# LeiXu84/fireFoam-dev

Hardware: AMD Instinct MI355X
Metric: PIMPLE outer-iterations/sec on 64M-cell hex mesh; pEqn SpMV GB/s vs HBM peak (higher is better)
Workload: dtype f64; 1 GPU; synthetic 400^3 hex box (64000000 cells), buoyant plume + 5-species EDC-shaped source, PIMPLE 1/2/0: rhoEqn + UEqn + YEEqn(4 Yi + h) + 2 pEqn per step; cells=64000000, faces=191520000, parallelism=1 GPU, transport_solvers=PBiCGStab+DILU

## Files before the change

firefoam-dev_amd/binding.py:

```python
import ctypes as C
import os
import re
import subprocess

import numpy as np

_HERE = os.path.dirname(os.path.abspath(__file__))
_ROOT = os.path.dirname(_HERE)
_SO = os.path.join(_HERE, "lib", "libffm.so")
_HDR = os.path.join(_ROOT, "include", "ffm.h")

SOLVERS = {"PCG": 0, "PBiCGStab": 1, "PBiCG": 2, "diagonal": 3, "smoothSolver": 4}
PRECONDS = {"none": 0, "DIC": 1, "DILU": 2, "GaussSeidel": 3, "symGaussSeidel": 4, "diagonal": 5}


class FfmError(RuntimeError):
    pass


class Perf(C.Structure):
    _fields_ = [("initialResidual", C.c_double), ("finalResidual", C.c_double),
                ("nIterations", C.c_int), ("converged", C.c_int), ("singular", C.c_int)]

    def as_dict(self):
# ... 69 lines not shown
        "ffm_ldu_bind_coeffs_native_d": ([vp, dp, dp, dp, C.c_int], C.c_int),
        "ffm_ldu_set_interfaces": ([vp, C.c_int, ip, C.POINTER(ip), C.POINTER(hp), C.POINTER(hp), ip], C.c_int),
        "ffm_ldu_set_global_cells": ([vp, C.c_long], C.c_int),
        "ffm_ldu_global_cells": ([vp], C.c_long),
        "ffm_spmv": ([vp, dp, dp], C.c_int),
        "ffm_tmul": ([vp, dp, dp], C.c_int),
        "ffm_sumA": ([vp, dp], C.c_int),
        "ffm_residual": ([vp, dp, dp, dp], C.c_int),
        "ffm_precond_setup": ([vp, C.c_int, dp], C.c_int),
        "ffm_precond_apply": ([vp, C.c_int, C.c_int, dp, dp], C.c_int),
        "ffm_precond_setup_multi": ([vp, C.c_int, C.c_int, C.POINTER(C.c_void_p), C.POINTER(C.c_void_p)], C.c_int),
        "ffm_ldu_tile_reach": ([vp, C.POINTER(C.c_int), C.POINTER(C.c_int), C.POINTER(C.c_int)], C.c_int),
        "ffm_gs_smooth": ([vp, C.c_int, C.c_int, dp, dp], C.c_int),
        "ffm_solve_d": ([vp, C.c_int, C.c_int, C.c_double, C.c_double, C.c_int, C.c_int, C.c_int, dp, dp,
                         C.POINTER(Perf)], C.c_int),
        "ffm_solve": ([vp, C.c_int, C.c_int, C.c_double, C.c_double, C.c_int, C.c_int, C.c_int, hp, hp,
                       C.POINTER(Perf)], C.c_int),
        "ffm_solve_multi_d": ([vp, C.c_int, C.c_int, C.c_int, C.c_double, C.c_double, C.c_int, C.c_int, C.POINTER(C.c_void_p), dp, dp,
                               C.POINTER(C.c_void_p), C.POINTER(C.c_void_p), C.POINTER(Perf)], C.c_int),
        "ffm_ldu_unbind_coeffs": ([vp], C.c_int),
        "ffm_ldu_offdiag_epoch": ([vp], C.c_ulong),
        "ffm_ldu_tile_coef_read": ([vp, C.c_int, hp], C.c_int),
        "ffm_ldu_tile_gathers": ([vp], C.c_long),
        "ffm_ldu_tile_code_bytes": ([vp, C.c_int, C.POINTER(C.c_long), C.POINTER(C.c_long)], C.c_int),
        "ffm_tile_share_codes": ([C.c_int, C.POINTER(C.c_long), ip, C.POINTER(C.c_ushort), C.c_long, C.c_int, C.c_long, C.POINTER(C.c_uint),
                                  C.POINTER(C.c_ushort), C.c_long, C.POINTER(C.c_long), C.POINTER(C.c_long)], C.c_int),
        "ffm_debug_pool_poison": ([vp, C.c_int], C.c_int),
        "ffm_bench_spmv": ([vp, dp, dp, C.c_int, hp], C.c_int),
        "ffm_bench_precond": ([vp, C.c_int, dp, dp, C.c_int, hp], C.c_int),
        "ffm_debug_set_sweep_ticket": ([vp, C.c_uint], C.c_int),
        "ffm_ldu_set_exchange_tags": ([vp, C.c_int, C.c_int, ip], C.c_int),
        "ffm_field_binary": ([vp, C.c_int, C.c_long, dp, dp, dp], C.c_int),
        "ffm_field_scalar": ([vp, C.c_int, C.c_long, dp, C.c_double, C.c_int, dp], C.c_int),
        "ffm_field_unary": ([vp, C.c_int, C.c_long, dp, dp], C.c_int),
        "ffm_field_eval": ([vp, C.c_long, C.c_int, C.POINTER(C.c_void_p), C.c_int, hp, C.c_int, C.POINTER(C.c_ushort), dp], C.c_int),
        "ffm_reduce_sum": ([vp, dp, C.c_long, hp], C.c_int),
        "ffm_reduce_min": ([vp, dp, C.c_long, hp], C.c_int),
        "ffm_reduce_max": ([vp, dp, C.c_long, hp], C.c_int),
        "ffm_reduce_dot": ([vp, dp, dp, C.c_long, hp], C.c_int),
        "ffm_reduce_summag": ([vp, dp, C.c_long, hp], C.c_int),
        "ffm_mesh_create": ([vp, hp, hp, hp, hp, hp, hp, C.c_int, ip, C.POINTER(ip), C.POINTER(hp), C.POINTER(hp), C.POINTER(vp)], C.c_int),
        "ffm_mesh_destroy": ([vp], C.c_int),
        "ffm_mesh_set_face_centres": ([vp, hp], C.c_int),
        "ffm_mesh_set_nonorth_correction": ([vp, hp], C.c_int),
        "ffm_pyro_create": ([vp, C.c_int, C.c_int, C.c_double, C.c_double, C.c_double, C.c_double, C.POINTER(vp)], C.c_int),
        "ffm_pyro_set_solids": ([vp, hp, hp], C.c_int),
# ... 484 lines not shown
    def face_map(self):
        m = np.empty(self.nFaces, np.int32)
        _check(lib().ffm_ldu_get_face_map(self.h, _ip(m)), "ffm_ldu_get_face_map")
        return m

    def bind_coeffs_native(self, diag, upper, lower=None, offDiagUnchanged=False):
        self._bound = (diag, upper, lower)
        _check(lib().ffm_ldu_bind_coeffs_native_d(self.h, C.c_void_p(diag.data_ptr()), C.c_void_p(upper.data_ptr()),
                                                  None if lower is None else C.c_void_p(lower.data_ptr()), 1 if offDiagUnchanged else 0),
               "ffm_ldu_bind_coeffs_native_d")
        return self

    def unbind_coeffs(self):
        _check(lib().ffm_ldu_unbind_coeffs(self.h), "ffm_ldu_unbind_coeffs")
        self._bound = None
        return self

    def tile_coef(self, which):
        self.ctx._ready()
        out = np.empty(3 * self.nOwned, np.float64)
        _check(lib().ffm_ldu_tile_coef_read(self.h, which, _hp(out)), "ffm_ldu_tile_coef_read")
        return out

    def tile_gathers(self):
        return int(lib().ffm_ldu_tile_gathers(self.h))

    def tile_code_bytes(self, which):
        u, t = C.c_long(), C.c_long()
        _check(lib().ffm_ldu_tile_code_bytes(self.h, which, C.byref(u), C.byref(t)), "ffm_ldu_tile_code_bytes")
        return u.value, t.value

    @property
    def offdiag_epoch(self):
        return int(lib().ffm_ldu_offdiag_epoch(self.h))

    def debug_set_sweep_ticket(self, value):
        _check(lib().ffm_debug_set_sweep_ticket(self.h, int(value) & 0xFFFFFFFF), "ffm_debug_set_sweep_ticket")

    @property
    def native_order(self):
        return bool(lib().ffm_ldu_is_native_order(self.h))

    def cell_order(self):
        o = np.empty(self.nCells, np.int32)
        _check(lib().ffm_ldu_get_cell_order(self.h, _ip(o)), "ffm_ldu_get_cell_order")
        return o
# ... 582 lines not shown
```

firefoam-dev_amd/csrc/ffm_internal.hpp:

```cpp
#pragma once
#include <hip/hip_runtime.h>
#include <string>
#include <tuple>
#include <unordered_map>

#include "ffm_host.hpp"

struct ncclComm;
struct ffm_tile_plan;

#define FFM_HIP(call)                                                            \
    do {                                                                         \
        hipError_t e_ = (call);                                                  \
        if (e_ != hipSuccess) {                                                  \
            ffm_set_error("%s:%d %s -> %s", __FILE__, __LINE__, #call,           \
                          hipGetErrorString(e_));                                \
            return FFM_ERR_HIP;                                                  \
        }                                                                        \
    } while (0)

constexpr int RED_THREADS = 256;
constexpr int RED_BLOCKS = 2048;
constexpr int NSCAL = 64;

// ... 96 lines not shown
    int upWidthUniform = -1;
    int loWidthUniform = -1;
    int maxW = 0;
    int loShift = 4;
    int *upOff = nullptr, *loOff = nullptr;
    int *upNbr = nullptr;
    int *loEnt = nullptr;
    int *flowOrder = nullptr;
    int *cellPerm = nullptr;
    int *faceSrc = nullptr;
    std::vector<int> h_callerToNative;
    std::vector<int> h_upOff, h_loOff, h_loEnt, h_upNbr;
    int *callerToNative = nullptr;

    double *diag = nullptr, *upper = nullptr, *lower = nullptr;
    double *lowerBuf = nullptr;

    int *rowSched = nullptr; int nSched = 0;

    double *rD = nullptr;
    int rDKind = -1;
    unsigned long coeffEpoch = 0, rDEpoch = ~0ul;
    unsigned long offDiagEpoch = 0;
    bool directPending = false;
    const double *directUpper = nullptr, *directLower = nullptr;
    unsigned long tileGathers = 0;
    double *diagBuf = nullptr, *upperBuf = nullptr;

    std::vector<double *> work;
    double *gsProd = nullptr;
    double *permIn[3] = {nullptr, nullptr, nullptr};

    std::vector<ffm_iface> ifaces;
    std::vector<int> ifaceTags, ghTags;
    int haloTotal = 0;
    int *ifFaceCells = nullptr;
    double *ifBou = nullptr, *ifInt = nullptr;
    double *haloSend = nullptr, *haloRecv = nullptr;
    double *haloSend_h = nullptr, *haloRecv_h = nullptr;
    int nIfCells = 0;
    int *ifCell = nullptr, *ifCellStart = nullptr, *ifItem = nullptr;

    std::vector<int> ghNbrRank, ghSendOff, ghRecvOff;
    int *ghSendCells = nullptr;
    bool ghPending = false;
    double *ghSendBuf = nullptr, *ghSendBuf_h = nullptr, *ghRecvBuf_h = nullptr;
// ... 32 lines not shown
int ffm_tile_gs_ghost_terms(ffm_ldu *A, const double *psi, double *bP);
int ffm_ghost_exchange(ffm_ldu *A, double *x);
int ffm_ghost_exchange_begin(ffm_ldu *A, double *x);
int ffm_ghost_exchange_split(ffm_ldu *A, const double *sendFrom, double *ghostInto);
int ffm_ghost_exchange_end(ffm_ldu *A);
int ffm_tile_gs(ffm_ldu *A, bool sym, double *psi, const double *bP, double *bSave, double *prod3);
bool ffm_tile_amul_usable(const ffm_ldu *A);
int ffm_tile_amul(ffm_ldu *A, const double *x, double *y, int dotSlot, const ffm_scal_op &t = ffm_scal_op());
void ffm_tile_free(ffm_ldu *A);
bool ffm_tile_usable(const ffm_ldu *A);
struct FfmFvSegs { int nSeg; const int4 *seg; const int4 *rec; };
bool ffm_tile_fv_segments(ffm_ldu *A, int runLength, FfmFvSegs *out);
bool ffm_tile_coef_direct_ok(const ffm_ldu *A);
int ffm_tile_coef_direct(ffm_ldu *A, bool lower, double **fU, double **fL, double **bU);
void ffm_tile_coef_written(ffm_ldu *A, const double *upper_d, const double *lower_d);
void ffm_tile_coef_adopt(ffm_ldu *A);
bool ffm_tile_pcg_fusable(const ffm_ldu *A);
int ffm_tile_pcg_fwd(ffm_ldu *A, double *rA, double *wA, int slot, const double *qA = nullptr, const ffm_scal_op &t = ffm_scal_op());
bool ffm_tile_amul_pcg_usable(const ffm_ldu *A);
bool ffm_tile_amul_asym_usable(const ffm_ldu *A);
int ffm_tile_amul_asym(ffm_ldu *A, const double *x, double *y);
int ffm_tile_amul_pcg(ffm_ldu *A, const double *w, const double *pin, double *pout, double *psi, double *y, int dotSlot, const ffm_scal_op &t = ffm_scal_op());
int ffm_tile_pcg_bwd(ffm_ldu *A, const double *rA, double *wA, int slot, const ffm_scal_op &t = ffm_scal_op());
#define FFM_TILE_MAXSYS 5
bool ffm_tile_multi_fits(const ffm_ldu *A, int n);
int ffm_tile_precond(ffm_ldu *A, int precond, bool transpose, int n, const double *const *rD, const double *const *r, double *const *w);
int ffm_tile_calc_rD(ffm_ldu *A, int n, const double *const *diag, double *const *D);
int ffm_k_spmv_multi(ffm_ldu *A, int n, const double *const *diag, const double *const *x, double *const *y, double *const *sumA);
extern "C" int ffm_solve_internal_i(ffm_ldu *A, int solver, int precond, double tol, double relTol, int minIter, int maxIter, int nSweeps,
                                    double *psi, const double *source, ffm_perf *perf);
int ffm_gs_smooth_i(ffm_ldu *A, bool sym, int nSweeps, double *psi, const double *b);
int ffm_halo_exchange(ffm_ldu *A, const double *x);
int ffm_ghost_exchange(ffm_ldu *A, double *x);
int ffm_read_scalars(ffm_ctx *ctx);

int ffm_k_dot(ffm_ctx *ctx, const double *x, const double *y, long n, int slot, const ffm_scal_op &t = ffm_scal_op());
int ffm_k_summag(ffm_ctx *ctx, const double *x, long n, int slot, const ffm_scal_op &t = ffm_scal_op());
int ffm_k_sum(ffm_ctx *ctx, const double *x, long n, int slot, const ffm_scal_op &t = ffm_scal_op());
int ffm_k_sumsqr(ffm_ctx *ctx, const double *x, long n, int slot, const ffm_scal_op &t = ffm_scal_op());

static inline int ffm_grid(long n, int threads) { return (int)((n + threads - 1) / threads); }
```

firefoam-dev_amd/csrc/ffm_ldu.hip:

```cpp
#include "ffm_internal.hpp"
#include "ffm_device.hpp"
#include <algorithm>

template <class T>
static int upload(ffm_ctx *c, T **dst, const std::vector<T> &v, size_t minCount = 1)
{
    size_t n = std::max(v.size(), minCount);
    FFM_HIP(hipMalloc((void **)dst, n * sizeof(T)));
    if (!v.empty()) FFM_HIP(hipMemcpyAsync(*dst, v.data(), v.size() * sizeof(T), hipMemcpyHostToDevice, c->stream));
    return FFM_OK;
}

extern "C" int ffm_ldu_create(ffm_ctx *ctx, int N, int F, const int *l, const int *u, ffm_ldu **out)
{ return ffm_ldu_create_ext(ctx, N, 0, F, l, u, out); }

extern "C" int ffm_ldu_create_ext(ffm_ctx *ctx, int nOwn, int nGhost, int F, const int *l, const int *u, ffm_ldu **out)
{ return ffm_ldu_create_hint(ctx, nOwn, nGhost, F, l, u, nullptr, out); }

static int ldu_create_impl(ffm_ctx *ctx, int nOwn, int nGhost, int F, const int *l, const int *u, const int *groupHint, int forceMode,
                           ffm_ldu **out);

extern "C" int ffm_ldu_create_hint(ffm_ctx *ctx, int nOwn, int nGhost, int F, const int *l, const int *u, const int *groupHint,
                                   ffm_ldu **out)
{
// ... 65 lines not shown
    A->nSlices = L.nSlices; A->upTotal = L.upTotal; A->loTotal = L.loTotal;
    A->upWidthUniform = L.upWidthUniform; A->loWidthUniform = L.loWidthUniform; A->maxW = L.maxW; A->loShift = L.loShift;
    A->h_upOff = L.upOff; A->h_loOff = L.loOff;
    A->h_callerToNative = std::move(L.callerToNative);
    const int rc = ldu_upload(A, a, L);
    if (rc) { ffm_ldu_destroy(A); return rc; }
    *out = A;
    return FFM_OK;
}

extern "C" int ffm_ldu_destroy(ffm_ldu *A)
{
    if (!A) return FFM_OK;
    hipSetDevice(A->ctx->device);
    hipStreamSynchronize(A->ctx->stream);
    for (double *w : A->work) hipFree(w);
    hipFree(A->gsProd);
    for (int i = 0; i < 3; i++) hipFree(A->permIn[i]);
    hipFree(A->upOff); hipFree(A->loOff); hipFree(A->upNbr); hipFree(A->loEnt); hipFree(A->faceSrc);
    hipFree(A->cellPerm); hipFree(A->callerToNative); hipFree(A->flowOrder);
    hipFree(A->grpCell); hipFree(A->sweepTicket); hipFree(A->rowSched);
    ffm_tile_free(A);
    hipFree(A->ghSendCells); hipFree(A->ghSendBuf); if (A->ghSendBuf_h) hipHostFree(A->ghSendBuf_h); if (A->ghRecvBuf_h) hipHostFree(A->ghRecvBuf_h);
    hipFree(A->diagBuf); hipFree(A->upperBuf); hipFree(A->lowerBuf); hipFree(A->rD);
    hipFree(A->ifFaceCells); hipFree(A->ifBou); hipFree(A->ifInt); hipFree(A->haloSend); hipFree(A->haloRecv);
    hipFree(A->ifCell); hipFree(A->ifCellStart); hipFree(A->ifItem);
    delete A;
    return FFM_OK;
}

extern "C" int ffm_ldu_ncells(const ffm_ldu *A) { return A ? A->nCells : FFM_ERR_ARG; }
extern "C" int ffm_ldu_sweep_mode(const ffm_ldu *A) { return !A ? FFM_ERR_ARG : A->sweepMode; }
extern "C" int ffm_ldu_nowned(const ffm_ldu *A) { return A ? A->nOwned : FFM_ERR_ARG; }
extern "C" int ffm_ldu_nfaces(const ffm_ldu *A) { return A ? A->nFaces : FFM_ERR_ARG; }
extern "C" int ffm_ldu_nlevels(const ffm_ldu *A) { return A ? A->nLevels : FFM_ERR_ARG; }
extern "C" int ffm_ldu_is_native_order(const ffm_ldu *A) { return A ? (A->identity ? 1 : 0) : FFM_ERR_ARG; }
extern "C" int ffm_ldu_get_cell_order(const ffm_ldu *A, int *newToOld)
{
    if (!A || !newToOld) return FFM_ERR_ARG;
    std::copy(A->h_newToOldCell.begin(), A->h_newToOldCell.end(), newToOld);
    return FFM_OK;
}
extern "C" int ffm_ldu_n_native_faces(const ffm_ldu *A) { return A ? A->upTotal : FFM_ERR_ARG; }
extern "C" int ffm_ldu_get_face_map(const ffm_ldu *A, int *callerToNative)
{
    if (!A || !callerToNative) return FFM_ERR_ARG;
    std::copy(A->h_callerToNative.begin(), A->h_callerToNative.end(), callerToNative);
// ... 419 lines not shown
```

firefoam-dev_amd/csrc/ffm_solve.hip:

```cpp
#include "ffm_internal.hpp"
#include "ffm_device.hpp"
#include <algorithm>
#include <cmath>
#include <cstring>


__global__ void k_scalar_op(double *s, int op, double arg, int iter, int in)
{
    if (threadIdx.x || blockIdx.x) return;
    scalar_op_body(s, op, arg, iter, in);
}

static int scalar_op(ffm_ctx *c, int op, double arg = 0.0, int iter = 0, int in = S_TMP0)
{
    hipLaunchKernelGGL(k_scalar_op, dim3(1), dim3(64), 0, c->stream, c->scal_d, op, arg, iter, in);
    FFM_HIP(hipGetLastError());
    return FFM_OK;
}
static ffm_scal_op tail_op(ffm_ctx *c, int op, double arg = 0.0, int iter = 0)
{
    ffm_scal_op t; t.op = op; t.arg = arg; t.iter = iter; t.fused = c->nRanks == 1 && !c->comm;
    return t;
}
static int finish_dot(ffm_ctx *c, const ffm_scal_op &t, int nSlots = 1)
// ... 346 lines not shown
        unsigned int z = 0;
        ffm_h2d(A->ctx, A->sweepTicket + 1, &z, sizeof(z));
        return FFM_ERR_HIP;
    }
    return FFM_OK;
}

static int calc_rD(ffm_ldu *A)
{
    if (A->sweepMode == 2) {
        const double *dg = A->diag;
        return ffm_tile_calc_rD(A, 1, &dg, &A->rD);
    }
    FlowArgs a; FFM_TRY(flow_args(A, SM_RD, a));
    FLOW_LAUNCH(SM_RD, a);
    FFM_HIP(hipGetLastError());
    return FFM_OK;
}

int ffm_precond_setup_i(ffm_ldu *A, int precond)
{
    if (A->rDKind == precond && A->rDEpoch == A->coeffEpoch) return FFM_OK;
    hipStream_t s = A->ctx->stream;
    switch (precond) {
    case FFM_NONE: break;
    case FFM_DIC:
        if (!A->symmetric) { ffm_set_error("DIC needs a symmetric matrix"); return FFM_ERR_UNSUPPORTED; }
        FFM_TRY(calc_rD(A)); break;
    case FFM_DILU: FFM_TRY(calc_rD(A)); break;
    case FFM_DIAGONALP:
        hipLaunchKernelGGL(k_recip, dim3(sgrid(A->nOwned)), dim3(256), 0, s, (long)A->nOwned, A->rD, A->diag);
        FFM_HIP(hipGetLastError());
        break;
    default: ffm_set_error("unknown preconditioner %d", precond); return FFM_ERR_UNSUPPORTED;
    }
    A->rDKind = precond; A->rDEpoch = A->coeffEpoch;
    return FFM_OK;
}

int ffm_precond_apply_i(ffm_ldu *A, int precond, bool transpose, const double *r, double *w)
{
    hipStream_t s = A->ctx->stream;
    const long N = A->nOwned;
    if (precond == FFM_NONE) { hipLaunchKernelGGL(k_copy, dim3(sgrid(N)), dim3(256), 0, s, N, w, r); FFM_HIP(hipGetLastError()); return FFM_OK; }
    if (precond == FFM_DIAGONALP) { hipLaunchKernelGGL(k_mul, dim3(sgrid(N)), dim3(256), 0, s, N, w, A->rD, r); FFM_HIP(hipGetLastError()); return FFM_OK; }
    if (A->sweepMode == 2) { const double *rD = A->rD; return ffm_tile_precond(A, precond, transpose, 1, &rD, &r, &w); }
// ... 71 lines not shown
    perf->initialResidual = c->scal_h[S_RES0];
    perf->finalResidual = perf->initialResidual;
    perf->nIterations = 0; perf->singular = 0; perf->converged = 0;
    return FFM_OK;
}

static int pcg(ffm_ldu *A, int precond, const Controls &k, double *psi, const double *source, ffm_perf *perf)
{
    ffm_ctx *c = A->ctx; hipStream_t s = c->stream; const long N = A->nOwned; const int g = sgrid(N);
    double *pA, *wA, *rA;
    FFM_TRY(ffm_ldu_work(A, 1, &pA)); FFM_TRY(ffm_ldu_work(A, 2, &wA)); FFM_TRY(ffm_ldu_work(A, 3, &rA));
    FFM_TRY(scalar_op(c, OP_RESET));
    FFM_TRY(ffm_k_spmv_sumA(A, psi, wA, pA));
    FFM_TRY(norm_and_initial(A, psi, source, wA, pA, rA, perf));
    if (k.minIter > 0 || !check_convergence(perf, k)) {
        FFM_TRY(ffm_precond_setup_i(A, precond));
        const ffm_scal_op beta = tail_op(c, OP_PCG_BETA), alpha = tail_op(c, OP_PCG_ALPHA), res = tail_op(c, OP_RES);
        if (precond == FFM_DIC && A->sweepMode == 2 && ffm_tile_pcg_fusable(A)) {
            const bool fuseP = ffm_tile_amul_pcg_usable(A);
            double *pB = nullptr, *qA = wA;
            if (fuseP) { FFM_TRY(ffm_ldu_work(A, 4, &pB)); FFM_TRY(ffm_ldu_work(A, 5, &qA)); }
            do {
                if (perf->nIterations == 0) {
                    FFM_TRY(ffm_precond_apply_i(A, precond, false, rA, wA));
                    FFM_TRY(ffm_k_dot(c, wA, rA, N, S_TMP0, beta));
                } else FFM_TRY(ffm_tile_pcg_bwd(A, rA, wA, S_TMP0, beta));
                FFM_TRY(finish_dot(c, beta));
                if (perf->nIterations == 0) {
                    hipLaunchKernelGGL(k_p_update, dim3(g), dim3(256), 0, s, N, pA, wA, c->scal_d, 1);
                    FFM_TRY(ffm_k_spmv_dot(A, pA, qA, S_TMP0, alpha));
                } else if (fuseP) {
                    FFM_TRY(ffm_tile_amul_pcg(A, wA, pA, pB, psi, qA, S_TMP0, alpha));
                    std::swap(pA, pB);
                } else {
                    hipLaunchKernelGGL(k_p_psi, dim3(g), dim3(256), 0, s, N, psi, pA, wA, c->scal_d);
                    FFM_TRY(ffm_k_spmv_dot(A, pA, qA, S_TMP0, alpha));
                }
                FFM_TRY(finish_dot(c, alpha));
                FFM_TRY(ffm_tile_pcg_fwd(A, rA, wA, S_TMP0, qA == wA ? nullptr : qA, res));
                FFM_TRY(finish_dot(c, res));
                FFM_TRY(ffm_read_scalars(c));
                if (c->scal_h[S_SING] != 0.0) { perf->singular = 1; break; }
                perf->finalResidual = c->scal_h[S_RES];
            } while ((++perf->nIterations < k.maxIter && !check_convergence(perf, k)) || perf->nIterations < k.minIter);
            if (!perf->singular) hipLaunchKernelGGL(k_axpy_alpha, dim3(g), dim3(256), 0, s, N, psi, pA, c->scal_d);
            FFM_HIP(hipGetLastError());
            return FFM_OK;
// ... 732 lines not shown
```

firefoam-dev_amd/csrc/ffm_tile.hip:

```cpp
#include "ffm_internal.hpp"
#include "ffm_device.hpp"
#include <algorithm>
#include <atomic>
#include <climits>

constexpr int T_RING = 4096;
constexpr int T_ENT = 256;
constexpr int T_THREADS = 256;
constexpr int T_W = FFM_TILE_W;
constexpr int T_PF = 8;
constexpr int T_PM = 3;
constexpr int T_XMAX = 64;
constexpr int T_RINGD = T_RING - 2 * T_ENT;
constexpr unsigned T_SPIN_LIMIT = 1u << 22;
constexpr unsigned T_NONE = 0xFFFFu;
constexpr int T_LDS = T_RING + 2 * T_XMAX + 1;
constexpr unsigned long long T_SENT = 0x7FF4DEADBEEFCAFEull;
static_assert(T_LDS < (int)T_NONE && T_ENT <= 256, "neighbour codes are LDS slots");
static_assert(T_PM >= 2 && T_PM < T_PF, "read-ahead distances");

struct TileDir {
    int nEnt = 0, nPub = 0;
    int *grpEnt = nullptr;
    int4 *rec = nullptr;
// ... 297 lines not shown
        T->nMail = (long)T->f.nPub + T->b.nPub + 2;
        FFM_HIP(hipMalloc((void **)&T->mailAll, sizeof(double) * T->nMail));
        T->f.mail = T->mailAll; T->b.mail = T->mailAll + T->f.nPub + 1;
        FfmStageTimer tm_("tile: amul plan");
        FFM_TRY(build_amul(A, grpOfCell, recF));
        if (!T->gsTables) T->usable = false;
    }
    return FFM_OK;
}

struct TileView {
    int G;
    const int *grpCell, *grpEnt, *extOff, *extSrc;
    const int4 *rec;
    const uint2 *code;
    unsigned int *ticket;
};

__device__ __forceinline__ double t_ld(const double *p) { return __hip_atomic_load(p, __ATOMIC_RELAXED, __HIP_MEMORY_SCOPE_AGENT); }
__device__ __forceinline__ void t_st(double *p, double v) { __hip_atomic_store(p, v, __ATOMIC_RELAXED, __HIP_MEMORY_SCOPE_AGENT); }
__device__ __forceinline__ void t_barrier() { asm volatile("s_waitcnt lgkmcnt(0)\n\ts_barrier" ::: "memory"); }
__device__ __forceinline__ bool t_pending(double v) { return (unsigned long long)__double_as_longlong(v) == T_SENT; }

enum { TM_FWD = 0, TM_BWD = 1, TM_RD = 2, TM_GSF = 3, TM_GSB = 4 };
struct __attribute__((aligned(8))) T3 { double a, b, c; };
static_assert(T_W == 3, "T3");

__device__ __noinline__ double t_wait_value(const double *addr, unsigned int *ticket, int *shAbort)
{
    double v = t_ld(addr);
    if (*(volatile int *)shAbort) return v;
    unsigned spins = 0;
    while (t_pending(v)) {
        __builtin_amdgcn_s_sleep(1);
        v = t_ld(addr);
        if ((++spins & 1023u) == 0u) {
            if (__hip_atomic_load(&ticket[1], __ATOMIC_RELAXED, __HIP_MEMORY_SCOPE_AGENT) != 0u) { *shAbort = 1; break; }
            if (spins > T_SPIN_LIMIT) { __hip_atomic_store(&ticket[1], 1u, __ATOMIC_RELAXED, __HIP_MEMORY_SCOPE_AGENT); *shAbort = 1; break; }
        }
    }
    return v;
}

constexpr int TM_PF = 4;
constexpr int TM_RING5 = 2048;
constexpr int tile_pf(int NF, int MODE) { return NF > 1 ? TM_PF : (MODE == TM_RD || MODE == TM_GSF) ? 6 : T_PF; }
static_assert(T_PM < TM_PF && tile_pf(1, TM_RD) <= T_PF && TM_PF <= T_PF, "read-ahead distances");
template <int NF> struct TileSys { const double *dg[NF]; const double *r[NF]; double *w[NF]; double *mail[NF]; };

template <int MODE, int NF, int R = T_RING, bool FUSE = false>
__global__ __launch_bounds__(T_THREADS + 64) void k_tile(TileView t, const double *__restrict__ ca, const double *__restrict__ cb, TileSys<NF> m,
                                                         double *aux = nullptr, const double *__restrict__ scal = nullptr, double *__restrict__ partials = nullptr)
{
    static_assert(R <= T_RING && (R & (R - 1)) == 0 && R > 2 * T_ENT, "ring length");
    static_assert(!FUSE || MODE == TM_FWD || MODE == TM_BWD, "fused vector updates: DIC/DILU application only");
    static_assert(MODE == TM_FWD || MODE == TM_BWD || MODE == TM_RD, "DILU / DIC application and calcReciprocalD (Gauss-Seidel: k_tile_gs)");
    static_assert(NF == 1 || !FUSE, "fused vector updates: one system");
    constexpr int LDS = R + 2 * T_XMAX + 1;
    constexpr bool ASC = MODE != TM_BWD;
    constexpr bool TWO = MODE == TM_RD;
    constexpr bool VEC = MODE != TM_RD;
    constexpr int W = T_W, PF = tile_pf(NF, MODE);
    __shared__ double ring[NF][LDS];
    __shared__ double shSum[4];
    __shared__ int4 shRec[4];
    __shared__ int shG;
    __shared__ int shAbort;
    const unsigned tid = threadIdx.x;
    if (tid == 0) {
        const unsigned tk = atomicAdd(&t.ticket[0], 1u);
        const int k = (int)(tk % (unsigned)t.G);
        shG = ASC ? k : t.G - 1 - k; shAbort = 0;
    }
    __syncthreads();
    const int g = __builtin_amdgcn_readfirstlane(shG);
    const unsigned gs = (unsigned)__builtin_amdgcn_readfirstlane(t.grpCell[g]);
    const int e0 = __builtin_amdgcn_readfirstlane(t.grpEnt[g]), e1 = __builtin_amdgcn_readfirstlane(t.grpEnt[g + 1]);
    if (e0 >= e1) { if (FUSE && tid == 0) partials[g] = 0.0; return; }

    if (tid >= (unsigned)T_THREADS) {
        const unsigned lane = tid - (unsigned)T_THREADS;
        int4 qrec[PF];
// ... 37 lines not shown
#undef Q_IDX
#undef Q_MAIL
#undef Q_PUT
        return;
    }

    unsigned pc[PF], ppb[PF];
    bool pok[PF];
    uint2 pq[PF];
    double pa[PF][W], pb[PF][TWO ? W : 1], pd[PF][NF], pv[PF][VEC ? NF : 1], pv2[FUSE ? PF : 1];
    double fsum = 0.0;
    const double fAlpha = (FUSE && MODE == TM_FWD) ? scal[S_ALPHA] : 0.0;
    const bool fSing = (FUSE && MODE == TM_FWD) ? (scal[S_SING] != 0.0) : false;
#define T_FETCH(k, e, R_) {                                                                             \
        const unsigned cnt_ = ((e) < e1) ? ((unsigned)R_.y & 0xFFFFu) : 0u;                              \
        const bool ok_ = tid < cnt_;                                                                     \
        const unsigned ps_ = ok_ ? (ASC ? tid : cnt_ - 1u - tid) : 0u;       \
        const unsigned cc_ = ok_ ? (unsigned)R_.x + ps_ : gs;                                            \
        const unsigned o8_ = cc_ * 8u, o24_ = cc_ * 24u;          \
        pq[k] = *(const uint2 *)((const char *)t.code + ((unsigned)R_.w + ps_ * 8u));                    \
        { const T3 v_ = *(const T3 *)((const char *)ca + o24_); pa[k][0] = v_.a; pa[k][1] = v_.b; pa[k][2] = v_.c; }     \
        if (TWO) { const T3 v_ = *(const T3 *)((const char *)cb + o24_); pb[k][0] = v_.a; pb[k][TWO ? 1 : 0] = v_.b; pb[k][TWO ? 2 : 0] = v_.c; } \
        _Pragma("unroll") for (int i_ = 0; i_ < NF; i_++) {                                              \
            pd[k][i_] = *(const double *)((const char *)m.dg[i_] + o8_);                                 \
            if (VEC) pv[k][VEC ? i_ : 0] = *(const double *)((const char *)((FUSE && MODE == TM_FWD) ? (const double *)aux : MODE == TM_BWD ? (const double *)m.w[i_] : m.r[i_]) + o8_); \
        }                                                                                                \
        if (FUSE) pv2[FUSE ? k : 0] = *(const double *)((const char *)((MODE == TM_FWD && !m.r[0]) ? (const double *)m.w[0] : m.r[0]) + o8_); \
        pc[k] = cc_; pok[k] = ok_; ppb[k] = (unsigned)R_.z;                                              \
    }
#pragma unroll
    for (int k = 0; k < PF; k++) { const int4 R0 = t.rec[min(e0 + k, e1)]; T_FETCH(k, e0 + k, R0); }
    t_barrier();
    for (int e = e0; e < e1; e += PF) {
#pragma unroll
        for (int k = 0; k < PF; k++) {
            const int ee = e + k;
            const int4 Rn = shRec[(ee + PF) & 3];
            {
                const unsigned c = pc[k];
                const unsigned cd[4] = {pq[k].x & 0xFFFFu, pq[k].x >> 16, pq[k].y & 0xFFFFu, pq[k].y >> 16};
                unsigned sl[W];
#pragma unroll
                for (int s = 0; s < W; s++)
                    sl[s] = (R == T_RING) ? min(cd[s], (unsigned)(LDS - 1))
                                          : (cd[s] < (unsigned)T_RING ? (cd[s] & (unsigned)(R - 1)) : min(cd[s] - (unsigned)(T_RING - R), (unsigned)(LDS - 1)));
                double val[NF];
#pragma unroll
                for (int i = 0; i < NF; i++) {
                    const double d = pd[k][i], v0 = VEC ? pv[k][VEC ? i : 0] : 0.0;
                    double x[W], v;
                    if (NF == 1) {
#pragma unroll
                        for (int s = 0; s < W; s++) x[s] = ring[i][sl[s]];
                    }
#define T_X(s) (NF == 1 ? x[s] : ring[i][sl[s]])
                    if (MODE == TM_FWD) {
                        double ri = v0;
                        if (FUSE) {
                            if (!fSing) { ri -= fAlpha * pv2[FUSE ? k : 0]; if (pok[k]) *(double *)((char *)aux + c * 8u) = ri; }
                            fsum += pok[k] ? fabs(ri) : 0.0;
                        }
                        v = d * ri;
#pragma unroll
                        for (int s = 0; s < W; s++) { const double nv = v - d * pa[k][s] * T_X(s); v = (cd[s] != T_NONE) ? nv : v; }
                    } else if (MODE == TM_BWD) {
                        v = v0;
#pragma unroll
                        for (int s = W - 1; s >= 0; s--) { const double nv = v - d * pa[k][s] * T_X(s); v = (cd[s] != T_NONE) ? nv : v; }
                    } else {
                        v = d;
#pragma unroll
                        for (int s = 0; s < W; s++) { const double nv = v - pa[k][s] * pb[k][TWO ? s : 0] / T_X(s); v = (cd[s] != T_NONE) ? nv : v; }
                    }
                    val[i] = v;
#undef T_X
                }
#define T_PUT(i) { *(double *)((char *)m.w[i] + c * 8u) = (MODE == TM_RD) ? 1.0 / val[i] : val[i]; ring[i][(c - gs) & (unsigned)(R - 1)] = val[i]; }
#define T_POST(i) { if (cd[3] != T_NONE) t_st(&m.mail[i][ppb[k] + cd[3]], val[i]); }
                if (NF == 1) {
                    if (pok[k]) T_PUT(0);
                    if (FUSE && MODE == TM_BWD) fsum += pok[k] ? val[0] * pv2[FUSE ? k : 0] : 0.0;
                    if (pok[k]) T_POST(0);
                } else if (pok[k]) {
#pragma unroll
                    for (int i = 0; i < NF; i++) { T_PUT(i); T_POST(i); }
                }
#undef T_PUT
#undef T_POST
            }
            T_FETCH(k, ee + PF, Rn);
            t_barrier();
        }
    }
#undef T_FETCH
    if (FUSE) {
        double v = fsum;
#pragma unroll
        for (int o = 32; o > 0; o >>= 1) v += __shfl_down(v, o, 64);
        if ((tid & 63u) == 0u) shSum[tid >> 6] = v;
        t_barrier();
        if (tid == 0) partials[g] = ((shSum[0] + shSum[1]) + shSum[2]) + shSum[3];
    }
}

// ... 272 lines not shown
    return FFM_OK;
}

__global__ void k_tile_sum_partials(int n, const double *__restrict__ partials, double *__restrict__ scal, int slot, ffm_scal_op t);
bool ffm_tile_pcg_fusable(const ffm_ldu *A)
{
    const char *e = getenv("FFM_PCG_UNFUSED");
    const bool off = e && atoi(e) != 0;
    return !off && ffm_tile_usable(A) && A->tile->G <= 4 * RED_BLOCKS;
}
int ffm_tile_pcg_fwd(ffm_ldu *A, double *rA, double *wA, int slot, const double *qA, const ffm_scal_op &t)
{
    ffm_tile_plan *T = A->tile;
    hipStream_t s = A->ctx->stream;
    const double *cf, *cb, *rD = A->rD; double *mail;
    FFM_TRY(tile_coef(A, T->f, true, &cf));
    FFM_TRY(tile_coef(A, T->b, true, &cb));
    FFM_TRY(tile_mail(A, 1, false, &mail));
    tile_launch<TM_FWD, 1, T_RING, true>(A, T->f, mail, cf, nullptr, &rD, &qA, &wA, rA, A->ctx->scal_d, A->ctx->partials_d);
    hipLaunchKernelGGL(k_tile_sum_partials, dim3(1), dim3(1024), 0, s, T->G, (const double *)A->ctx->partials_d, A->ctx->scal_d, slot, t);
    FFM_HIP(hipGetLastError());
    return FFM_OK;
}
int ffm_tile_pcg_bwd(ffm_ldu *A, const double *rA, double *wA, int slot, const ffm_scal_op &t)
{
    ffm_tile_plan *T = A->tile;
    hipStream_t s = A->ctx->stream;
    const double *cb, *rD = A->rD;
    FFM_TRY(tile_coef(A, T->b, true, &cb));
    tile_launch<TM_BWD, 1, T_RING, true>(A, T->b, T->mailAll, cb, nullptr, &rD, &rA, &wA, nullptr, A->ctx->scal_d, A->ctx->partials_d);
    hipLaunchKernelGGL(k_tile_sum_partials, dim3(1), dim3(1024), 0, s, T->G, (const double *)A->ctx->partials_d, A->ctx->scal_d, slot, t);
    FFM_HIP(hipGetLastError());
    return FFM_OK;
}

__global__ void k_tile_gs_products(long n3, const int *__restrict__ nbrCell, const double *__restrict__ coef, const double *__restrict__ psi,
                                   double *__restrict__ out)
{
    for (long i = (long)blockIdx.x * blockDim.x + threadIdx.x; i < n3; i += (long)gridDim.x * blockDim.x) {
        const int nb = nbrCell[i];
        out[i] = (nb >= 0) ? coef[i] * psi[nb] : 0.0;
    }
}

int ffm_tile_gs(ffm_ldu *A, bool sym, double *psi, const double *bP, double *bSave, double *prod)
{
    ffm_tile_plan *T = A->tile;
    hipStream_t s = A->ctx->stream;
    const double *cl, *cu; double *mail;
    FFM_TRY(tile_coef(A, T->f, A->lower == A->upper, &cl));
    FFM_TRY(tile_coef(A, T->b, true, &cu));
    const long n3 = (long)T_W * A->nOwned;
    hipLaunchKernelGGL(k_tile_gs_products, dim3(std::max(1, std::min(ffm_grid(n3, 256), 8 * RED_BLOCKS))), dim3(256), 0, s, n3,
// ... 274 lines not shown
```

include/ffm.h:

```cpp
#ifndef FFM_H
#define FFM_H

#include <stddef.h>
#include <stdint.h>

#ifdef __cplusplus
extern "C" {
#endif

typedef struct ffm_ctx ffm_ctx;
typedef struct ffm_ldu ffm_ldu;

typedef enum ffm_status {
    FFM_OK = 0,
    FFM_ERR_ARG = -1,
    FFM_ERR_ADDR = -2,
    FFM_ERR_HIP = -3,
    FFM_ERR_NODEVICE = -4,
    FFM_ERR_UNSUPPORTED = -5,
    FFM_ERR_COMM = -6
} ffm_status;

typedef enum ffm_solver {
    FFM_PCG = 0, FFM_PBICGSTAB = 1, FFM_PBICG = 2, FFM_DIAGONAL = 3, FFM_SMOOTH = 4,
// ... 62 lines not shown
int ffm_ldu_sweep_mode(const ffm_ldu *ldu);
int ffm_ldu_is_native_order(const ffm_ldu *ldu);
int ffm_ldu_get_cell_order(const ffm_ldu *ldu, int *newToOld);

int ffm_renumber_levels(int nCells, int nFaces, const int *lowerAddr,
                        const int *upperAddr, int *newToOldCell,
                        int *newToOldFace);

int ffm_ldu_set_coeffs(ffm_ldu *ldu, const double *diag, const double *upper,
                       const double *lower);
int ffm_ldu_set_coeffs_d(ffm_ldu *ldu, const double *diag_d,
                         const double *upper_d, const double *lower_d);

int ffm_ldu_n_native_faces(const ffm_ldu *ldu);
int ffm_ldu_get_face_map(const ffm_ldu *ldu, int *callerToNative);
int ffm_ldu_set_coeffs_native_d(ffm_ldu *ldu, const double *diag_d,
                                const double *upper_d, const double *lower_d);
int ffm_ldu_bind_coeffs_native_d(ffm_ldu *ldu, const double *diag_d, const double *upper_d,
                                 const double *lower_d, int offDiagUnchanged);
int ffm_ldu_unbind_coeffs(ffm_ldu *ldu);
unsigned long ffm_ldu_offdiag_epoch(const ffm_ldu *ldu);
int ffm_ldu_tile_coef_read(ffm_ldu *ldu, int which, double *out_h);
long ffm_ldu_tile_gathers(const ffm_ldu *ldu);
int ffm_ldu_tile_code_bytes(const ffm_ldu *ldu, int which, long *uniqueBytes, long *totalBytes);
int ffm_tile_share_codes(int nBlocks, const long *start, const int *len, const unsigned short *codes, long nCodes, int share, long padShorts,
                         unsigned int *offset_out, unsigned short *pool_out, long poolCapacity, long *uniqueShorts, long *poolShorts);

int ffm_ldu_set_interfaces(ffm_ldu *ldu, int nPatches, const int *patchSizes,
                           const int *const *faceCells,
                           const double *const *bouCoeffs,
                           const double *const *intCoeffs,
                           const int *neighbRank);
int ffm_ldu_set_global_cells(ffm_ldu *ldu, long globalCells);
long ffm_ldu_global_cells(const ffm_ldu *ldu);
int ffm_ldu_set_exchange_tags(ffm_ldu *ldu, int kind, int n, const int *tags);

int ffm_spmv(ffm_ldu *ldu, const double *x_d, double *y_d);
int ffm_tmul(ffm_ldu *ldu, const double *x_d, double *y_d);
int ffm_sumA(ffm_ldu *ldu, double *s_d);
int ffm_residual(ffm_ldu *ldu, const double *x_d, const double *b_d, double *r_d);
int ffm_precond_setup(ffm_ldu *ldu, int precond, double *rD_out_d );
int ffm_precond_apply(ffm_ldu *ldu, int precond, int transpose,
                      const double *r_d, double *w_d);
int ffm_precond_setup_multi(ffm_ldu *ldu, int precond, int nSys, const double *const *diag_d, double *const *rD_out_d);
int ffm_ldu_tile_reach(const ffm_ldu *ldu, int *reach, int *limit, int *limit5);
int ffm_gs_smooth(ffm_ldu *ldu, int symmetric_sweep, int nSweeps, double *psi_d,
// ... 368 lines not shown
```

Measured before the change: 3.424 outer-iterations/s.

## Cache rD-scaled backward DIC coefficients and reuse them in PCG backward sweeps

On the first PCG preconditioner application, the backward DIC sweep now also stores the products rD*coef for each cell's three neighbours into a new per-matrix buffer. Later fused backward sweeps read this pre-scaled triple instead of the separate rD array and the coefficients, which drops one stream and one multiply per neighbour. The buffer is tied to the coefficient epoch so it is invalidated when the matrix changes. The cost is extra memory of three doubles per cell, an extra write on the first iteration, and a device-allocation path. The behaviour can be turned off with an environment variable.

```diff
diff --git a/firefoam-dev_amd/binding.py b/firefoam-dev_amd/binding.py
--- a/firefoam-dev_amd/binding.py
+++ b/firefoam-dev_amd/binding.py
@@ -115,6 +115,7 @@
         "ffm_ldu_offdiag_epoch": ([vp], C.c_ulong),
         "ffm_ldu_tile_coef_read": ([vp, C.c_int, hp], C.c_int),
         "ffm_ldu_tile_gathers": ([vp], C.c_long),
+        "ffm_ldu_dic_scaled_read": ([vp, hp, hp], C.c_int),
         "ffm_ldu_tile_code_bytes": ([vp, C.c_int, C.POINTER(C.c_long), C.POINTER(C.c_long)], C.c_int),
         "ffm_tile_share_codes": ([C.c_int, C.POINTER(C.c_long), ip, C.POINTER(C.c_ushort), C.c_long, C.c_int, C.c_long, C.POINTER(C.c_uint),
                                   C.POINTER(C.c_ushort), C.c_long, C.POINTER(C.c_long), C.POINTER(C.c_long)], C.c_int),
@@ -645,6 +646,12 @@
         _check(lib().ffm_ldu_tile_coef_read(self.h, which, _hp(out)), "ffm_ldu_tile_coef_read")
         return out
 
+    def dic_scaled(self):
+        self.ctx._ready()
+        cbS, rD = np.empty(3 * self.nOwned, np.float64), np.empty(self.nOwned, np.float64)
+        _check(lib().ffm_ldu_dic_scaled_read(self.h, _hp(cbS), _hp(rD)), "ffm_ldu_dic_scaled_read")
+        return cbS, rD
+
     def tile_gathers(self):
         return int(lib().ffm_ldu_tile_gathers(self.h))
 
diff --git a/firefoam-dev_amd/csrc/ffm_internal.hpp b/firefoam-dev_amd/csrc/ffm_internal.hpp
--- a/firefoam-dev_amd/csrc/ffm_internal.hpp
+++ b/firefoam-dev_amd/csrc/ffm_internal.hpp
@@ -142,6 +142,8 @@
     int rDKind = -1;
     unsigned long coeffEpoch = 0, rDEpoch = ~0ul;
     unsigned long offDiagEpoch = 0;
+    double *cbS = nullptr;
+    unsigned long cbSEpoch = ~0ul;
     bool directPending = false;
     const double *directUpper = nullptr, *directLower = nullptr;
     unsigned long tileGathers = 0;
@@ -220,6 +222,8 @@
 int ffm_tile_amul_asym(ffm_ldu *A, const double *x, double *y);
 int ffm_tile_amul_pcg(ffm_ldu *A, const double *w, const double *pin, double *pout, double *psi, double *y, int dotSlot, const ffm_scal_op &t = ffm_scal_op());
 int ffm_tile_pcg_bwd(ffm_ldu *A, const double *rA, double *wA, int slot, const ffm_scal_op &t = ffm_scal_op());
+bool ffm_tile_dic_scaled(const ffm_ldu *A);
+int ffm_tile_precond_dic_scaled(ffm_ldu *A, const double *r, double *w);
 #define FFM_TILE_MAXSYS 5
 bool ffm_tile_multi_fits(const ffm_ldu *A, int n);
 int ffm_tile_precond(ffm_ldu *A, int precond, bool transpose, int n, const double *const *rD, const double *const *r, double *const *w);
diff --git a/firefoam-dev_amd/csrc/ffm_ldu.hip b/firefoam-dev_amd/csrc/ffm_ldu.hip
--- a/firefoam-dev_amd/csrc/ffm_ldu.hip
+++ b/firefoam-dev_amd/csrc/ffm_ldu.hip
@@ -111,7 +111,7 @@
     hipFree(A->grpCell); hipFree(A->sweepTicket); hipFree(A->rowSched);
     ffm_tile_free(A);
     hipFree(A->ghSendCells); hipFree(A->ghSendBuf); if (A->ghSendBuf_h) hipHostFree(A->ghSendBuf_h); if (A->ghRecvBuf_h) hipHostFree(A->ghRecvBuf_h);
-    hipFree(A->diagBuf); hipFree(A->upperBuf); hipFree(A->lowerBuf); hipFree(A->rD);
+    hipFree(A->diagBuf); hipFree(A->upperBuf); hipFree(A->lowerBuf); hipFree(A->rD); hipFree(A->cbS);
     hipFree(A->ifFaceCells); hipFree(A->ifBou); hipFree(A->ifInt); hipFree(A->haloSend); hipFree(A->haloRecv);
     hipFree(A->ifCell); hipFree(A->ifCellStart); hipFree(A->ifItem);
     delete A;
diff --git a/firefoam-dev_amd/csrc/ffm_solve.hip b/firefoam-dev_amd/csrc/ffm_solve.hip
--- a/firefoam-dev_amd/csrc/ffm_solve.hip
+++ b/firefoam-dev_amd/csrc/ffm_solve.hip
@@ -392,6 +392,7 @@
 {
     if (A->rDKind == precond && A->rDEpoch == A->coeffEpoch) return FFM_OK;
     hipStream_t s = A->ctx->stream;
+    A->cbSEpoch = ~0ul;
     switch (precond) {
     case FFM_NONE: break;
     case FFM_DIC:
@@ -509,7 +510,7 @@
             if (fuseP) { FFM_TRY(ffm_ldu_work(A, 4, &pB)); FFM_TRY(ffm_ldu_work(A, 5, &qA)); }
             do {
                 if (perf->nIterations == 0) {
-                    FFM_TRY(ffm_precond_apply_i(A, precond, false, rA, wA));
+                    FFM_TRY(ffm_tile_precond_dic_scaled(A, rA, wA));
                     FFM_TRY(ffm_k_dot(c, wA, rA, N, S_TMP0, beta));
                 } else FFM_TRY(ffm_tile_pcg_bwd(A, rA, wA, S_TMP0, beta));
                 FFM_TRY(finish_dot(c, beta));
diff --git a/firefoam-dev_amd/csrc/ffm_tile.hip b/firefoam-dev_amd/csrc/ffm_tile.hip
--- a/firefoam-dev_amd/csrc/ffm_tile.hip
+++ b/firefoam-dev_amd/csrc/ffm_tile.hip
@@ -343,7 +343,7 @@
 __device__ __forceinline__ void t_barrier() { asm volatile("s_waitcnt lgkmcnt(0)\n\ts_barrier" ::: "memory"); }
 __device__ __forceinline__ bool t_pending(double v) { return (unsigned long long)__double_as_longlong(v) == T_SENT; }
 
-enum { TM_FWD = 0, TM_BWD = 1, TM_RD = 2, TM_GSF = 3, TM_GSB = 4 };
+enum { TM_FWD = 0, TM_BWD = 1, TM_RD = 2, TM_GSF = 3, TM_GSB = 4, TM_BWDW = 5, TM_BWDS = 6 };
 struct __attribute__((aligned(8))) T3 { double a, b, c; };
 static_assert(T_W == 3, "T3");
 
@@ -374,11 +374,15 @@
                                                          double *aux = nullptr, const double *__restrict__ scal = nullptr, double *__restrict__ partials = nullptr)
 {
     static_assert(R <= T_RING && (R & (R - 1)) == 0 && R > 2 * T_ENT, "ring length");
-    static_assert(!FUSE || MODE == TM_FWD || MODE == TM_BWD, "fused vector updates: DIC/DILU application only");
-    static_assert(MODE == TM_FWD || MODE == TM_BWD || MODE == TM_RD, "DILU / DIC application and calcReciprocalD (Gauss-Seidel: k_tile_gs)");
+    constexpr bool BWD = MODE == TM_BWD || MODE == TM_BWDW || MODE == TM_BWDS;
+    constexpr bool DG = MODE != TM_BWDS;
+    static_assert(!FUSE || MODE == TM_FWD || MODE == TM_BWD || MODE == TM_BWDS, "fused vector updates: DIC/DILU application only");
+    static_assert(MODE == TM_FWD || BWD || MODE == TM_RD, "DILU / DIC application and calcReciprocalD (Gauss-Seidel: k_tile_gs)");
     static_assert(NF == 1 || !FUSE, "fused vector updates: one system");
+    static_assert(NF == 1 || (MODE != TM_BWDW && MODE != TM_BWDS), "the scaled triple: one system");
+    static_assert(MODE != TM_BWDW || !FUSE, "the scaled triple is stored through aux");
     constexpr int LDS = R + 2 * T_XMAX + 1;
-    constexpr bool ASC = MODE != TM_BWD;
+    constexpr bool ASC = !BWD;
     constexpr bool TWO = MODE == TM_RD;
     constexpr bool VEC = MODE != TM_RD;
     constexpr int W = T_W, PF = tile_pf(NF, MODE);
@@ -462,8 +466,8 @@
         { const T3 v_ = *(const T3 *)((const char *)ca + o24_); pa[k][0] = v_.a; pa[k][1] = v_.b; pa[k][2] = v_.c; }     \
         if (TWO) { const T3 v_ = *(const T3 *)((const char *)cb + o24_); pb[k][0] = v_.a; pb[k][TWO ? 1 : 0] = v_.b; pb[k][TWO ? 2 : 0] = v_.c; } \
         _Pragma("unroll") for (int i_ = 0; i_ < NF; i_++) {                                              \
-            pd[k][i_] = *(const double *)((const char *)m.dg[i_] + o8_);                                 \
-            if (VEC) pv[k][VEC ? i_ : 0] = *(const double *)((const char *)((FUSE && MODE == TM_FWD) ? (const double *)aux : MODE == TM_BWD ? (const double *)m.w[i_] : m.r[i_]) + o8_); \
+            if (DG) pd[k][i_] = *(const double *)((const char *)m.dg[i_] + o8_);                         \
+            if (VEC) pv[k][VEC ? i_ : 0] = *(const double *)((const char *)((FUSE && MODE == TM_FWD) ? (const double *)aux : BWD ? (const double *)m.w[i_] : m.r[i_]) + o8_); \
         }                                                                                                \
         if (FUSE) pv2[FUSE ? k : 0] = *(const double *)((const char *)((MODE == TM_FWD && !m.r[0]) ? (const double *)m.w[0] : m.r[0]) + o8_); \
         pc[k] = cc_; pok[k] = ok_; ppb[k] = (unsigned)R_.z;                                              \
@@ -484,10 +488,10 @@
                 for (int s = 0; s < W; s++)
                     sl[s] = (R == T_RING) ? min(cd[s], (unsigned)(LDS - 1))
                                           : (cd[s] < (unsigned)T_RING ? (cd[s] & (unsigned)(R - 1)) : min(cd[s] - (unsigned)(T_RING - R), (unsigned)(LDS - 1)));
-                double val[NF];
+                double val[NF], ds[W];
 #pragma unroll
                 for (int i = 0; i < NF; i++) {
-                    const double d = pd[k][i], v0 = VEC ? pv[k][VEC ? i : 0] : 0.0;
+                    const double d = DG ? pd[k][i] : 0.0, v0 = VEC ? pv[k][VEC ? i : 0] : 0.0;
                     double x[W], v;
                     if (NF == 1) {
 #pragma unroll
@@ -503,10 +507,13 @@
                         v = d * ri;
 #pragma unroll
                         for (int s = 0; s < W; s++) { const double nv = v - d * pa[k][s] * T_X(s); v = (cd[s] != T_NONE) ? nv : v; }
-                    } else if (MODE == TM_BWD) {
+                    } else if (BWD) {
                         v = v0;
 #pragma unroll
-                        for (int s = W - 1; s >= 0; s--) { const double nv = v - d * pa[k][s] * T_X(s); v = (cd[s] != T_NONE) ? nv : v; }
+                        for (int s = W - 1; s >= 0; s--) {
+                            ds[s] = DG ? d * pa[k][s] : pa[k][s];
+                            const double nv = v - ds[s] * T_X(s); v = (cd[s] != T_NONE) ? nv : v;
+                        }
                     } else {
                         v = d;
 #pragma unroll
@@ -518,8 +525,8 @@
 #define T_PUT(i) { *(double *)((char *)m.w[i] + c * 8u) = (MODE == TM_RD) ? 1.0 / val[i] : val[i]; ring[i][(c - gs) & (unsigned)(R - 1)] = val[i]; }
 #define T_POST(i) { if (cd[3] != T_NONE) t_st(&m.mail[i][ppb[k] + cd[3]], val[i]); }
                 if (NF == 1) {
-                    if (pok[k]) T_PUT(0);
-                    if (FUSE && MODE == TM_BWD) fsum += pok[k] ? val[0] * pv2[FUSE ? k : 0] : 0.0;
+                    if (pok[k]) { T_PUT(0); if (MODE == TM_BWDW) *(T3 *)((char *)aux + c * 24u) = T3{ds[0], ds[1], ds[2]}; }
+                    if (FUSE && BWD) fsum += pok[k] ? val[0] * pv2[FUSE ? k : 0] : 0.0;
                     if (pok[k]) T_POST(0);
                 } else if (pok[k]) {
 #pragma unroll
@@ -838,13 +845,47 @@
     FFM_HIP(hipGetLastError());
     return FFM_OK;
 }
+bool ffm_tile_dic_scaled(const ffm_ldu *A)
+{
+    const char *e = getenv("FFM_DIC_SCALED");
+    return !(e && atoi(e) == 0) && ffm_tile_pcg_fusable(A);
+}
+static bool dic_scaled_valid(const ffm_ldu *A)
+{
+    return A->cbS && A->rDKind == FFM_DIC && A->rDEpoch == A->coeffEpoch && A->cbSEpoch == A->coeffEpoch;
+}
+int ffm_tile_precond_dic_scaled(ffm_ldu *A, const double *r, double *w)
+{
+    ffm_tile_plan *T = A->tile;
+    if (!ffm_tile_dic_scaled(A) || dic_scaled_valid(A)) { const double *rD = A->rD; return ffm_tile_precond(A, FFM_DIC, false, 1, &rD, &r, &w); }
+    if (!A->cbS) FFM_HIP(hipMalloc((void **)&A->cbS, sizeof(double) * (size_t)T_W * (size_t)std::max(A->nOwned, 1)));
+    const double *cf, *cb, *rD = A->rD; double *mail;
+    FFM_TRY(tile_coef(A, T->f, true, &cf));
+    FFM_TRY(tile_coef(A, T->b, true, &cb));
+    FFM_TRY(tile_mail(A, 1, false, &mail));
+    tile_launch<TM_FWD, 1>(A, T->f, mail, cf, nullptr, &rD, &r, &w);
+    tile_launch<TM_BWDW, 1>(A, T->b, mail, cb, nullptr, &rD, nullptr, &w, A->cbS);
+    FFM_HIP(hipGetLastError());
+    A->cbSEpoch = A->coeffEpoch;
+    return FFM_OK;
+}
+extern "C" int ffm_ldu_dic_scaled_read(ffm_ldu *A, double *cbS_h, double *rD_h)
+{
+    if (!A || !cbS_h || !rD_h) return FFM_ERR_ARG;
+    if (!ffm_tile_usable(A) || !dic_scaled_valid(A)) { ffm_set_error("ffm_ldu_dic_scaled_read: the matrix holds no current scaled triple"); return FFM_ERR_UNSUPPORTED; }
+    FFM_TRY(ffm_d2h(A->ctx, cbS_h, A->cbS, sizeof(double) * (size_t)T_W * A->nOwned));
+    return ffm_d2h(A->ctx, rD_h, A->rD, sizeof(double) * (size_t)A->nOwned);
+}
 int ffm_tile_pcg_bwd(ffm_ldu *A, const double *rA, double *wA, int slot, const ffm_scal_op &t)
 {
     ffm_tile_plan *T = A->tile;
     hipStream_t s = A->ctx->stream;
     const double *cb, *rD = A->rD;
     FFM_TRY(tile_coef(A, T->b, true, &cb));
-    tile_launch<TM_BWD, 1, T_RING, true>(A, T->b, T->mailAll, cb, nullptr, &rD, &rA, &wA, nullptr, A->ctx->scal_d, A->ctx->partials_d);
+    if (ffm_tile_dic_scaled(A) && dic_scaled_valid(A))
+        tile_launch<TM_BWDS, 1, T_RING, true>(A, T->b, T->mailAll, A->cbS, nullptr, &rD, &rA, &wA, nullptr, A->ctx->scal_d, A->ctx->partials_d);
+    else
+        tile_launch<TM_BWD, 1, T_RING, true>(A, T->b, T->mailAll, cb, nullptr, &rD, &rA, &wA, nullptr, A->ctx->scal_d, A->ctx->partials_d);
     hipLaunchKernelGGL(k_tile_sum_partials, dim3(1), dim3(1024), 0, s, T->G, (const double *)A->ctx->partials_d, A->ctx->scal_d, slot, t);
     FFM_HIP(hipGetLastError());
     return FFM_OK;
diff --git a/include/ffm.h b/include/ffm.h
--- a/include/ffm.h
+++ b/include/ffm.h
@@ -108,6 +108,7 @@
 unsigned long ffm_ldu_offdiag_epoch(const ffm_ldu *ldu);
 int ffm_ldu_tile_coef_read(ffm_ldu *ldu, int which, double *out_h);
 long ffm_ldu_tile_gathers(const ffm_ldu *ldu);
+int ffm_ldu_dic_scaled_read(ffm_ldu *ldu, double *cbS_h, double *rD_h);
 int ffm_ldu_tile_code_bytes(const ffm_ldu *ldu, int which, long *uniqueBytes, long *totalBytes);
 int ffm_tile_share_codes(int nBlocks, const long *start, const int *len, const unsigned short *codes, long nCodes, int share, long padShorts,
                          unsigned int *offset_out, unsigned short *pool_out, long poolCapacity, long *uniqueShorts, long *poolShorts);
```

Measured after the change: 3.458 outer-iterations/s (median of 6 runs). No clear change (+1.0%).
